# neonnnnn/nimfm

Measured on AMD Instinct MI355X. Metric: SGD training samples/sec/epoch, higher is better.
Workload: dtype f64

## Files before the change

nimfm_amd/csrc/mb.h:

```cpp
#pragma once
#include <functional>
#include <vector>

#include "opt_views.h"
#include "plan.h"

namespace nfm {

struct MbWork {
  DevBuf Abuf;
  DevBuf rec;
  DevBuf partsA;
  DevBuf partsB;
  DevBuf Dtab;
  DevBuf Stab;
  DevBuf Ftab;
  DevBuf out_acc;
  DevBuf contrib;
  DevBuf itbuf;
  DevBuf hpart;
  DevBuf prox;
  bool use_graph = true;
  void* graph_exec = nullptr;
  uint64_t graph_plan_serial = 0;
  uint64_t graph_data_serial = 0;
  int graph_opt = -1;
  int64_t batch_begin = 0, batch_end = -1;
  std::function<int(int64_t)> after_batch;
  std::function<bool(int64_t)> is_sync;
  std::vector<void*> seg_execs;
  std::vector<int64_t> seg_cut;
  uint64_t seg_plan_serial = 0, seg_data_serial = 0;
  int seg_opt = -1;
  int64_t seg_key = -1;
// ... 17 lines not shown
```

nimfm_amd/csrc/mb_fm.hip:

```cpp
#include "mb_fm_kernels.h"

namespace nfm {

#define NFM_DECL(LL) \
  int mb_fm_run_L##LL(nfm_ctx* ctx, int opt_kind, bool gen, const CsrView& X, const ModelView& M, const OptView& O, const Plan& P, MbWork& W, int TA);
NFM_DECL(1) NFM_DECL(2) NFM_DECL(4) NFM_DECL(8) NFM_DECL(16) NFM_DECL(32) NFM_DECL(64)
#undef NFM_DECL


__global__ void k_schedule(OptView O, int fit_linear, int fit_intercept, const int64_t* __restrict__ bat_pos,
                           const double* __restrict__ it0p, double* __restrict__ Dtab ,
                           double* __restrict__ Ftab ) {
  __shared__ double red[3][kBlock];
  const double it0 = *it0p;
  const int b = blockIdx.x;
  const int64_t p0 = bat_pos[b], p1 = bat_pos[b + 1];
  double dP = 1.0, dw = 1.0, d0 = 1.0;
  for (int64_t p = p0 + threadIdx.x; p < p1; p += kBlock) {
    const double it = it0 + (double)p;
    dP *= 1 - dev::get_eta(O.sched, O.eta0, O.power, O.beta, it) * O.beta;
    if (fit_linear) dw *= 1 - dev::get_eta(O.sched, O.eta0, O.power, O.alpha, it) * O.alpha;
    if (fit_intercept) d0 *= 1 - dev::get_eta(O.sched, O.eta0, O.power, O.alpha0, it) * O.alpha0;
  }
  red[0][threadIdx.x] = dP;
// ... 98 lines not shown
  const hipError_t e2 = hipGraphInstantiate(&exec, graph, nullptr, nullptr, 0);
  (void)hipGraphDestroy(graph);
  NFM_HIP_CHECK(e2);
  seg_execs.push_back(exec);
  seg_cut.push_back(b);
  NFM_HIP_CHECK(hipGraphLaunch(exec, ctx->stream));
  return NFM_OK;
}
int MbWork::seg_resume(nfm_ctx* ctx) {
  NFM_HIP_CHECK(hipStreamBeginCapture(ctx->stream, hipStreamCaptureModeThreadLocal));
  return NFM_OK;
}
MbWork::~MbWork() { drop_graph(); }

int mb_fm_epoch(nfm_ctx* ctx, int opt_kind, const CsrView& X, const ModelView& M, const OptView& O, const Plan& P, MbWork& W,
                int64_t it0, double* out2_host, uint64_t data_serial, bool defer_sync) {
  NFM_CHECK(M.kind == NFM_KIND_FM, NFM_ERR_UNSUPPORTED, "mb_fm_epoch: FM only");
  NFM_CHECK(M.degree <= dev::kMaxDeg, NFM_ERR_UNSUPPORTED, "mini-batch mode supports degree <= %d", dev::kMaxDeg);
  NFM_CHECK(M.Kp == 2 * M.L && M.Kp <= 128, NFM_ERR_UNSUPPORTED, "mini-batch mode: factor blocks of at most 128 (api.hip splits wider FMs)");
  hipStream_t st = ctx->stream;
  int TA = 0;
  for (int o = 0; o < M.nb; ++o) TA += M.deg_of(o) - 1;
  constexpr int kMinGroupsPerBlock = kWavesPerBlock;
  const void* before[] = {W.Abuf.p, W.rec.p, W.partsA.p, W.partsB.p, W.Dtab.p, W.Stab.p, W.Ftab.p, W.out_acc.p, W.itbuf.p, W.hpart.p, W.prox.p};
  NFM_TRY(W.Abuf.ensure(sizeof(double) * (size_t)std::max<int64_t>(P.max_batch, 1) * std::max(TA, 1) * M.Kp));
  NFM_TRY(W.rec.ensure(sizeof(SampleRec) * (size_t)std::max<int64_t>(P.max_batch, 1)));
  NFM_TRY(W.partsA.ensure(sizeof(PartA) * (size_t)(P.max_batch / 2 + 2)));
  NFM_TRY(W.partsB.ensure(sizeof(double) * 2 * (size_t)(P.max_unique / kMinGroupsPerBlock + P.max_batch / kWavesPerBlock + P.max_heavy / kWavesPerBlock + 6)));
  NFM_TRY(W.hpart.ensure(sizeof(double) * (size_t)std::max<int64_t>(P.max_segs, 1) * std::max(M.nb, 1) * (2 * M.Kp + 4)));
  NFM_TRY(W.Dtab.ensure(sizeof(double) * 4 * (size_t)(P.n_batches + 1)));
  NFM_TRY(W.Stab.ensure(sizeof(double) * 2 * (size_t)(P.n_batches + 1)));
  NFM_TRY(W.Ftab.ensure(sizeof(double) * 2 * kFtab * (size_t)(P.n_batches + 1)));
  NFM_TRY(W.out_acc.ensure(sizeof(double) * 2));
  NFM_TRY(W.itbuf.ensure(sizeof(double)));
  if (opt_kind == OPT_PSGD)
    NFM_TRY(W.prox.ensure(sizeof(double) * ((size_t)M.nb * M.da + (size_t)std::max(M.nb, 1) * M.Kp * (3 + 2 * 1024) + 8)));
  const void* after[] = {W.Abuf.p, W.rec.p, W.partsA.p, W.partsB.p, W.Dtab.p, W.Stab.p, W.Ftab.p, W.out_acc.p, W.itbuf.p, W.hpart.p, W.prox.p};
  for (size_t q = 0; q < sizeof(before) / sizeof(before[0]); ++q)
    if (before[q] != after[q]) W.drop_graph();
  hipLaunchKernelGGL(k_set_double, dim3(1), dim3(1), 0, st, W.itbuf.as<double>(), (double)it0);
  const bool want_graph = W.use_graph && !W.after_batch && !ctx->timing.enabled && !P.has_perm && P.n_batches >= 8;
  if (want_graph) {
    if (!W.graph_exec || W.graph_plan_serial != P.serial || W.graph_opt != opt_kind || W.graph_data_serial != data_serial) {
      W.drop_graph();
      hipGraph_t graph = nullptr;
      NFM_HIP_CHECK(hipStreamBeginCapture(st, hipStreamCaptureModeThreadLocal));
      const int rc = enqueue_epoch(ctx, opt_kind, X, M, O, P, W, TA);
      const hipError_t e = hipStreamEndCapture(st, &graph);
      if (rc != NFM_OK) {
        if (graph) (void)hipGraphDestroy(graph);
        return rc;
      }
      NFM_HIP_CHECK(e);
      hipGraphExec_t exec = nullptr;
      const hipError_t e2 = hipGraphInstantiate(&exec, graph, nullptr, nullptr, 0);
      (void)hipGraphDestroy(graph);
      NFM_HIP_CHECK(e2);
      W.graph_exec = exec;
      W.graph_plan_serial = P.serial;
      W.graph_data_serial = data_serial;
// ... 60 lines not shown
```

nimfm_amd/csrc/mb_fm_kernels.h:

```cpp
#pragma once
#include "fm_device.h"
#include "mb.h"

namespace nfm {

#ifndef NFM_WAVE_STAGE2
#define NFM_WAVE_STAGE2 1
#endif
#ifndef NFM_COL_MINW
#define NFM_COL_MINW 1
#endif
#ifndef NFM_COL_D3
#define NFM_COL_D3 1
#endif
#ifndef NFM_REG_NTSEL
#define NFM_REG_NTSEL 0
#endif
#ifndef NFM_ADA2_MINW
#define NFM_ADA2_MINW 2
#endif

struct SampleRec {
  double dL, etaP, etaw, yhat;
};
// ... 1 lines not shown
  double loss, viol, acc0, acc1;
};

static_assert(sizeof(SampleRec) == 32 && sizeof(PartA) == 32, "record layout");

constexpr int kFtab = 64;

struct RowArgs {
  CsrView X;
  ModelView M;
  OptView O;
  const int64_t* perm;
  int64_t begin, p0;
  int32_t len, use_stored, TA, nt;
  double it_b;
  const double* it0p;
  const double* scales;
  const double* scales_n;
  const int64_t* toff;
  const uint8_t* single;
  double* Abuf;
  SampleRec* rec;
  PartA* parts;
};

__device__ __forceinline__ void st_nt(double* p, double2 v) {
  dev::v2d_t w;
  w.x = v.x;
  w.y = v.y;
  __builtin_nontemporal_store(w, reinterpret_cast<dev::v2d_t*>(p));
}
__device__ __forceinline__ double2 ld_nt(const double* p) {
  const dev::v2d_t v = __builtin_nontemporal_load(reinterpret_cast<const dev::v2d_t*>(p));
  return double2{v.x, v.y};
}
template <bool NT>
__device__ __forceinline__ void st_row(double* p, double2 v) {
  if (NT) st_nt(p, v);
  else *reinterpret_cast<double2*>(p) = v;
}
template <bool NT>
__device__ __forceinline__ double2 ld_row(const double* p) {
  if (NT) return ld_nt(p);
  return *reinterpret_cast<const double2*>(p);
}
template <int L, int SPLIT, bool GEN, class PS>
// ... 423 lines not shown
    } else {
      const dev::AdaParams ps{O.G, O.N, O.eta0, O.eta0 * itp * O.beta};
      part += row_forward<L, SPLIT, GEN>(ps, X, M, q0, m, m_tot, slot, l, lane, valid, Arow, A1);
    }
  }
#pragma unroll
  for (int s = 1; s < LPS; s <<= 1) part += dev::shfl_xor_d(part, s);
  double dL, yh_w = 0.0;
  if (SPW == 1 && NFM_WAVE_STAGE2) {
    const double yh = wave_uniform(b0 + part);
    yh_w = yh;
    dL = wave_uniform(dev::loss_grad(O.loss, O.loss_param, y, yh));
    double r_acc0 = 0.0, r_acc1 = 0.0;
    if (OPT == OPT_SGD) {
      if (M.fit_intercept) {
        r_acc0 = eta_b * dL;
        r_acc1 = eta_b;
      }
    } else if (M.fit_intercept) {
      r_acc0 = dL;
      r_acc1 = dL * dL;
    }
    if (lane == 0) {
      if (valid) a.rec[pib] = SampleRec{dL, etaP, etaw, yh};
      s_dL[sib] = valid ? r_acc0 : 0.0;
      s_etaP[sib] = valid ? r_acc1 : 0.0;
    }
  } else {
  if (slot == 0 && l == 0) {
    s_y[sib] = y;
    s_yh[sib] = b0 + part;
  }
  __syncthreads();
  if (wv == 0) {
    double r_loss = 0.0, r_acc0 = 0.0, r_acc1 = 0.0;
    for (int t = lane; t < SPB; t += kWave) {
      const int pt = blockIdx.x * SPB + t;
      if (pt < a.len) {
        const double yt = s_y[t], yh = s_yh[t];
        const double dL = dev::loss_grad(O.loss, O.loss_param, yt, yh);
        r_loss += dev::loss_value(O.loss, O.loss_param, yt, yh);
        double etaP = 0.0, etaw = 0.0;
        if (OPT == OPT_SGD) {
          const double it = (a.it0p[0] + a.it_b) + (double)pt;
          etaP = dev::get_eta(O.sched, O.eta0, O.power, O.beta, it);
          etaw = dev::get_eta(O.sched, O.eta0, O.power, O.alpha, it);
          if (M.fit_intercept) {
            const double eta0 = dev::get_eta(O.sched, O.eta0, O.power, O.alpha0, it);
            r_acc0 += eta0 * dL;
            r_acc1 += eta0;
          }
        } else if (M.fit_intercept) {
          r_acc0 += dL;
          r_acc1 += dL * dL;
        }
        a.rec[pt] = SampleRec{dL, etaP, etaw, yh};
        s_dL[t] = dL;
        s_etaP[t] = etaP;
        s_etaw[t] = etaw;
      }
    }
    r_loss = dev::wave_sum(r_loss);
    r_acc0 = dev::wave_sum(r_acc0);
    r_acc1 = dev::wave_sum(r_acc1);
    if (lane == 0) {
      s_part[0] = r_loss;
      s_part[2] = r_acc0;
      s_part[3] = r_acc1;
    }
  }
  __syncthreads();
  dL = s_dL[sib];
  etaP = s_etaP[sib];
  etaw = s_etaw[sib];
  }
  double r_viol = 0.0;
  if (HELD && a.single != nullptr) {
    const double sP = OPT == OPT_SGD ? a.scales[0] : 1.0, sw = OPT == OPT_SGD ? a.scales[1] : 1.0;
    const double sPn = OPT == OPT_SGD ? a.scales_n[0] : 1.0, swn = OPT == OPT_SGD ? a.scales_n[1] : 1.0;
// ... 191 lines not shown
    a1.x += tx;
    a1.y += ty;
    a2.x += tx * tx;
    a2.y += ty * ty;
    __builtin_amdgcn_sched_barrier(0);
  }
#pragma unroll
  for (int s = 16; s < kWave; s <<= 1) {
    a1.x += dev::shfl_xor_d(a1.x, s);
    a1.y += dev::shfl_xor_d(a1.y, s);
    a2.x += dev::shfl_xor_d(a2.x, s);
    a2.y += dev::shfl_xor_d(a2.y, s);
  }
  if (valid && slot == 0) *reinterpret_cast<double2*>(a.Abuf + (size_t)pib * a.TA * M.Kp + eoff) = a1;
  if (slot == 0) part += (a1.x * a1.x - a2.x) / 2 + (a1.y * a1.y - a2.y) / 2;
  part = dev::wave_sum(part);
  if (lane == 0) s_part[sib][half] = part;
  __syncthreads();
  double b0 = M.sc[SC_INTERCEPT];
  if (M.fit_intercept) b0 = -O.eta0 * O.gsc[0] / (sqrt(O.gsc[1]) + O.eta0 * itp * O.alpha0);
  const double yh = wave_uniform(b0 + (s_part[sib][0] + s_part[sib][1]));
  const double dL = wave_uniform(dev::loss_grad(O.loss, O.loss_param, y, yh));
  if (half == 0 && lane == 0) {
    if (valid) a.rec[pib] = SampleRec{dL, 0.0, 0.0, yh};
    s_acc0[sib] = (valid && M.fit_intercept) ? dL : 0.0;
    s_acc1[sib] = (valid && M.fit_intercept) ? dL * dL : 0.0;
  }
  asm volatile("" : "+v"(jq), "+v"(fq), "+v"(xq));
  double r_viol = 0.0;
#ifndef NFM_ADA2_V
#define NFM_ADA2_V 8
#endif
  constexpr int V = NFM_ADA2_V;
#pragma unroll
  for (int u0 = 0; u0 < NU; u0 += V) {
    int f[V], j[V];
    double xv[V];
    double2 po[V];
#pragma unroll
    for (int u = 0; u < V; ++u) {
      f[u] = lane_bcast_i<SPLIT>(fq, u0 + u, slot);
      j[u] = lane_bcast_i<SPLIT>(jq, u0 + u, slot);
      xv[u] = lane_bcast_d<SPLIT>(xq, u0 + u, slot);
    }
    if (O.track_viol) {
#pragma unroll
      for (int u = 0; u < V; ++u) {
// ... 59 lines not shown
  int64_t begin, p0;
  int32_t len_i, nS;
  const int32_t* ucol;
  const int64_t* uptr;
  const int32_t* ucol_s;
  const int64_t* ubeg_s;
  const int32_t* ucnt_s;
  const int32_t* tpos;
  const double* tx;
  int64_t u0, u1;
  const double* scales_b;
  const double* scales_n;
  const double* Dtab_b;
  const double* Ftab_b;
  const double* Abuf;
  const SampleRec* rec;
  double* parts;
  const PartA* partsA;
  const double* parts_prev;
  double* out_acc;
  double it_b, len;
  const double* it0p;
  int32_t TA, use_stored, nA, n_prev;
};

struct WAcc {
  double a0 = 0.0, a1 = 0.0;
};

template <int OPT, bool GEN, int TU, int LG, int MODE>
__device__ __forceinline__ double col_block(const ColArgs& a, size_t e, int deg, int slot, int l, int64_t t0, int64_t t1,
                                            double sP, double sPn, double fP, bool do_w, WAcc& wacc, double c_total = 0.0,
                                            double* hp = nullptr, int64_t nseg = 0, int PW = 0, int seg_stride = 0) {
  const ModelView& M = a.M;
  const OptView& O = a.O;
  double viol = 0.0;
  double2 stored = {0.0, 0.0}, g2 = {0.0, 0.0}, n2 = {0.0, 0.0}, p;
  if (OPT == OPT_SGD) {
    stored = dev::ld_stream(M.P + e);
    p.x = sP * stored.x;
    p.y = sP * stored.y;
  } else if (OPT == OPT_PSGD) {
    stored = dev::ld_stream(M.P + e);
    p = stored;
  } else {
    g2 = dev::ld_stream(O.G + e);
// ... 965 lines not shown
      s1[f] = load_stage(h1[f]);
    }
#pragma unroll
    for (int f = 0; f < NF; ++f) finish(h0[f], s0[f], G[f]);
#pragma unroll
    for (int f = 0; f < NF; ++f) {
      h0[f] = h1[f];
      h1[f] = h2[f];
      s0[f] = s1[f];
    }
  }
  viol = dev::wave_sum(viol);
  if (lane == 0) red[0][wv] = viol;
  __syncthreads();
  if (threadIdx.x == 0) {
    double v = 0.0;
    for (int w_ = 0; w_ < kWavesPerBlock; ++w_) v += red[0][w_];
    a.parts[a.nS + blockIdx.x] = v;
  }
  if (!closer) return;
  col_closer<OPT>(a, red);
}

__global__ void k_epoch_close(const double* __restrict__ parts, int n, double* __restrict__ out_acc);

template <int L, int SPLIT, int OPT, bool GEN>
static void launch_row(hipStream_t st, const RowArgs& ra, int mode, int n_cu, int* n_blocks) {
  const bool sing = ra.single != nullptr;
  constexpr int SPW = kWave / (L * SPLIT);
  const int nA = (ra.len + kWavesPerBlock * SPW - 1) / (kWavesPerBlock * SPW);
  *n_blocks = nA;
  constexpr bool CAN_HOLD = held_entries<L, SPLIT>() > 0;
  constexpr bool CAN_REG = CAN_HOLD && !GEN && OPT == OPT_SGD && L * SPLIT == kWave;
  if (CAN_REG && mode == 2 && ra.nt)
    hipLaunchKernelGGL((k_row_phase<L, SPLIT, OPT, GEN, (CAN_REG ? 4 : 0), false>), dim3(nA), dim3(kBlock), 0, st, ra);
  else if (CAN_REG && mode == 2)
    hipLaunchKernelGGL((k_row_phase<L, SPLIT, OPT, GEN, (CAN_REG ? 2 : 0), false>), dim3(nA), dim3(kBlock), 0, st, ra);
  else if (CAN_HOLD && mode == 3)
    hipLaunchKernelGGL((k_row_phase<L, SPLIT, OPT, GEN, (CAN_HOLD ? 3 : 0), false>), dim3(nA), dim3(kBlock), 0, st, ra);
  else if (CAN_HOLD && mode >= 1)
    hipLaunchKernelGGL((k_row_phase<L, SPLIT, OPT, GEN, (CAN_HOLD ? 1 : 0), false>), dim3(nA), dim3(kBlock), 0, st, ra);
  else if (sing && !GEN)
    hipLaunchKernelGGL((k_row_phase<L, SPLIT, OPT, GEN, 0, !GEN>), dim3(nA), dim3(kBlock), 0, st, ra);
  else
    hipLaunchKernelGGL((k_row_phase<L, SPLIT, OPT, GEN, 0, false>), dim3(nA), dim3(kBlock), 0, st, ra);
}

static int held_capacity(int L, int s) {
  const int lps = L * s;
  const int e = lps >= kWave ? 1 : (lps >= 8 ? (kWave / lps > 4 ? 4 : kWave / lps) : 0);
  return e * lps;
}

template <int L, int OPT, bool GEN>
static int run_batches(nfm_ctx* ctx, const CsrView& X, const ModelView& M, const OptView& O, const Plan& P, MbWork& W,
                       int TA) {
  constexpr int R = kWave / L;
  hipStream_t st = ctx->stream;
  const double* Stab = W.Stab.as<double>();
  const double* Dtab = W.Dtab.as<double>();
  const double* it0p = W.itbuf.as<double>();
  const double avg_row = X.n > 0 ? (double)X.nnz / (double)X.n + M.n_aug : 0.0;
  const size_t partsB_half = W.partsB.bytes / sizeof(double) / 2;
  const char* tu_env = getenv("NFM_TU");
  const int tu = tu_env ? atoi(tu_env) : 2;
  const bool have_singles = !GEN && P.use_singles;
  static const int stream_env = getenv("NFM_STREAM") ? atoi(getenv("NFM_STREAM")) : -1;
  const size_t table_bytes = sizeof(double) * (size_t)M.nb * M.da * M.Kp * (OPT == OPT_ADAGRAD ? 3 : 1);
  const bool stream_rows = stream_env >= 0 ? stream_env != 0 : (have_singles && table_bytes > ((size_t)384 << 20));
  static const bool env_kernel = getenv("NFM_SINGLES_KERNEL") && atoi(getenv("NFM_SINGLES_KERNEL")) != 0;
  const bool singles_in_row = have_singles && !env_kernel;
  const bool singles_in_col = have_singles && !singles_in_row;
  int n_prev = 0;
  const int64_t b_first = std::min(W.batch_begin, P.n_batches), b_last = W.batch_end < 0 ? P.n_batches : std::min(W.batch_end, P.n_batches);
  for (int64_t b = b_first; b < b_last; ++b) {
    const int64_t p0 = P.bat_pos[b];
    const int len = (int)(P.bat_pos[b + 1] - p0);
    const int use_stored = (OPT == OPT_PSGD || (OPT == OPT_ADAGRAD && P.first_singleton && b == 0)) ? 1 : 0;
    const double it_b = OPT == OPT_PSGD ? (double)b : (double)p0;
    constexpr int ROPT = OPT == OPT_PSGD ? OPT_ADAGRAD : OPT;
    const int split = choose_split(L, len, avg_row, ctx->n_cu);
    auto mode_for = [&](int s_used) {
      static const bool held_on = !(getenv("NFM_HELD") && atoi(getenv("NFM_HELD")) == 0);
      static const bool reg_on = !(getenv("NFM_NQ") && atoi(getenv("NFM_NQ")) == 0);
      if (!held_on || held_capacity(L, s_used) == 0 || M.nb == 0) return 0;
      if (X.max_row + M.n_aug > held_capacity(L, s_used)) return 3;
      if (!GEN && reg_on && OPT == OPT_SGD && singles_in_row && L * s_used == kWave) return 2;
      return 1;
    };
    int nA;
    {
      RowArgs ra{X, M, O, P.has_perm ? P.perm.as<int64_t>() : nullptr, P.begin, p0, len, use_stored, TA, stream_rows ? 1 : 0, it_b, it0p,
                 OPT == OPT_SGD ? Stab + 2 * b : M.sc, OPT == OPT_SGD ? Stab + 2 * (b + 1) : M.sc,
                 singles_in_row ? P.toff.as<int64_t>() : nullptr,
                 singles_in_row ? P.single.as<uint8_t>() : nullptr, W.Abuf.as<double>(), W.rec.as<SampleRec>(),
                 W.partsA.as<PartA>()};
      TimedLaunch tl(ctx, "row_phase");
      int s_used;
      static const bool ada2_on = !(getenv("NFM_ADA2") && atoi(getenv("NFM_ADA2")) == 0);
      if (OPT == OPT_ADAGRAD && !GEN && L == 32 && ada2_on && singles_in_row && !use_stored && X.max_row + M.n_aug <= 64) {
        nA = (len + 1) / 2;
        if (stream_rows)
          hipLaunchKernelGGL((k_row_phase_ada2<OPT_ADAGRAD, true>), dim3(nA), dim3(kBlock), 0, st, ra);
        else
          hipLaunchKernelGGL((k_row_phase_ada2<OPT_ADAGRAD, false>), dim3(nA), dim3(kBlock), 0, st, ra);
        s_used = 2;
      } else
      if (R >= 16 && split >= 16) { launch_row<L, (R >= 16 ? 16 : R), ROPT, GEN>(st, ra, mode_for(R >= 16 ? 16 : R), ctx->n_cu, &nA); s_used = R >= 16 ? 16 : R; }
      else if (R >= 8 && split >= 8) { launch_row<L, (R >= 8 ? 8 : R), ROPT, GEN>(st, ra, mode_for(R >= 8 ? 8 : R), ctx->n_cu, &nA); s_used = R >= 8 ? 8 : R; }
      else if (R >= 4 && split >= 4) { launch_row<L, (R >= 4 ? 4 : R), ROPT, GEN>(st, ra, mode_for(R >= 4 ? 4 : R), ctx->n_cu, &nA); s_used = R >= 4 ? 4 : R; }
      else if (R >= 2 && split >= 2) { launch_row<L, (R >= 2 ? 2 : R), ROPT, GEN>(st, ra, mode_for(R >= 2 ? 2 : R), ctx->n_cu, &nA); s_used = R >= 2 ? 2 : R; }
      else { launch_row<L, 1, ROPT, GEN>(st, ra, mode_for(1), ctx->n_cu, &nA); s_used = 1; }
      (void)s_used;
    }
    const int64_t u0 = P.bat_uoff[b], u1 = P.bat_uoff[b + 1];
    const int per_block = kWavesPerBlock * R;
    int nB = (int)((u1 - u0 + per_block - 1) / per_block);
    static const bool col_pipe_env = !(getenv("NFM_COL_PIPE") && atoi(getenv("NFM_COL_PIPE")) == 0);
    const bool col_pipe = col_pipe_env && !GEN && M.nb == 1 && OPT != OPT_PSGD;
    static const int col_occ = [] {
      int nb_ = 0, np_ = 0;
      if (hipOccupancyMaxActiveBlocksPerMultiprocessor(&nb_, k_col_phase<L, OPT, GEN, 2, true>, kBlock, 0) != hipSuccess || nb_ < 1) nb_ = 8;
      if (!GEN && OPT != OPT_PSGD && col_pipe_env &&
          hipOccupancyMaxActiveBlocksPerMultiprocessor(&np_, k_col_sparse<L, (OPT == OPT_PSGD ? OPT_SGD : OPT)>, kBlock, 0) == hipSuccess && np_ >= 1)
        nb_ = np_;
      return nb_;
    }();
    static const int col_wg_per_cu = getenv("NFM_COL_WG") ? atoi(getenv("NFM_COL_WG")) : col_occ;
    static const int cap_sets = getenv("NFM_COL_CAP_SETS") ? atoi(getenv("NFM_COL_CAP_SETS")) : 4;
    const bool nB_capped = tu == 2 && col_wg_per_cu > 0 && nB > cap_sets * ctx->n_cu * col_wg_per_cu;
    if (nB_capped) nB = ctx->n_cu * col_wg_per_cu;
    nB += 1;
    const int nS = singles_in_col ? (len + kWavesPerBlock - 1) / kWavesPerBlock : 0;
    double* parts_cur = W.partsB.as<double>() + (b & 1) * partsB_half;
    const double* parts_prev = W.partsB.as<double>() + ((b + 1) & 1) * partsB_half;
    {
      ColArgs ca{X, M, O, P.has_perm ? P.perm.as<int64_t>() : nullptr, singles_in_col ? P.toff.as<int64_t>() : nullptr,
                 singles_in_col ? P.single.as<uint8_t>() : nullptr, P.begin, p0, len, nS,
                 P.ucol.as<int32_t>(), P.uptr.as<int64_t>(), P.ucol_s.as<int32_t>(), P.ubeg_s.as<int64_t>(), P.ucnt_s.as<int32_t>(),
                 P.tpos.as<int32_t>(), P.tx.as<double>(), u0, u1,
                 OPT == OPT_SGD ? Stab + 2 * b : M.sc, OPT == OPT_SGD ? Stab + 2 * (b + 1) : M.sc,
                 OPT == OPT_SGD ? Dtab + 4 * b : nullptr,
                 OPT == OPT_SGD ? W.Ftab.as<double>() + (size_t)b * 2 * kFtab : nullptr, W.Abuf.as<double>(),
                 W.rec.as<SampleRec>(), parts_cur, W.partsA.as<PartA>(), parts_prev, W.out_acc.as<double>(), it_b,
                 (double)len, it0p, TA, use_stored, nA, n_prev};
      if (nS > 0) {
        TimedLaunch tls(ctx, "singles");
        hipLaunchKernelGGL((k_singles<L, OPT>), dim3(nS), dim3(kBlock), 0, st, ca);
      }
      TimedLaunch tl(ctx, "col_phase");
      const bool strided = nB_capped;
      if (tu == 1 && OPT != OPT_PSGD)
        hipLaunchKernelGGL((k_col_phase<L, (OPT == OPT_PSGD ? OPT_SGD : OPT), GEN, 1, false>), dim3(nB), dim3(kBlock), 0, st, ca);
      else if (tu == 4 && OPT != OPT_PSGD)
        hipLaunchKernelGGL((k_col_phase<L, (OPT == OPT_PSGD ? OPT_SGD : OPT), GEN, 4, false>), dim3(nB), dim3(kBlock), 0, st, ca);
      else if (strided && col_pipe)
        hipLaunchKernelGGL((k_col_sparse<L, (OPT == OPT_PSGD ? OPT_SGD : OPT)>), dim3(nB), dim3(kBlock), 0, st, ca);
      else if (strided)
        hipLaunchKernelGGL((k_col_phase<L, OPT, GEN, 2, true>), dim3(nB), dim3(kBlock), 0, st, ca);
      else
        hipLaunchKernelGGL((k_col_phase<L, OPT, GEN, 2, false>), dim3(nB), dim3(kBlock), 0, st, ca);
    }
    int nH = 0;
    if (M.nb > 0 && P.bat_hoff[b + 1] > P.bat_hoff[b]) {
      const int PW = 2 * M.Kp + 4;
      HeavyArgs ha{P.hv_u.as<int64_t>(), P.hv_seg0.as<int64_t>(), P.bat_hoff[b], P.bat_hoff[b + 1], P.bat_soff[b],
                   P.bat_soff[b + 1], W.hpart.as<double>(), parts_cur + nS + nB, PW, 0};
      ColArgs ca{X, M, O, P.has_perm ? P.perm.as<int64_t>() : nullptr, nullptr, nullptr, P.begin, p0, len, nS,
                 P.ucol.as<int32_t>(), P.uptr.as<int64_t>(), P.ucol_s.as<int32_t>(), P.ubeg_s.as<int64_t>(), P.ucnt_s.as<int32_t>(),
                 P.tpos.as<int32_t>(), P.tx.as<double>(), u0, u1,
                 OPT == OPT_SGD ? Stab + 2 * b : M.sc, OPT == OPT_SGD ? Stab + 2 * (b + 1) : M.sc,
                 OPT == OPT_SGD ? Dtab + 4 * b : nullptr,
                 OPT == OPT_SGD ? W.Ftab.as<double>() + (size_t)b * 2 * kFtab : nullptr, W.Abuf.as<double>(),
                 W.rec.as<SampleRec>(), parts_cur, W.partsA.as<PartA>(), parts_prev, W.out_acc.as<double>(), it_b,
                 (double)len, it0p, TA, use_stored, nA, n_prev};
      const int nsb = (int)((ha.s1 - ha.s0 + per_block - 1) / per_block);
      nH = (int)((ha.h1 - ha.h0 + kWavesPerBlock - 1) / kWavesPerBlock);
      {
        TimedLaunch tl(ctx, "heavy_partial");
        hipLaunchKernelGGL((k_heavy_partial<L, OPT, GEN>), dim3(nsb), dim3(kBlock), 0, st, ca, ha);
      }
      TimedLaunch tl(ctx, "heavy_apply");
      hipLaunchKernelGGL((k_heavy_apply<L, OPT, GEN>), dim3(nH), dim3(kBlock), 0, st, ca, ha);
    }
    n_prev = nB + nS + nH;
    if (OPT == OPT_PSGD && O.gradP == nullptr) launch_psgd_step(ctx, M, O, W, it0p, it_b);
    if (W.after_batch) {
      const bool cut = W.seg_recording && W.is_sync && W.is_sync(b);
      if (cut) NFM_TRY(W.seg_cut_here(ctx, b));
      NFM_TRY(W.after_batch(b));
      if (cut) NFM_TRY(W.seg_resume(ctx));
    }
  }
  if (b_last > b_first) {
    const double* parts_last = W.partsB.as<double>() + ((b_last - 1) & 1) * partsB_half;
    hipLaunchKernelGGL(k_epoch_close, dim3(1), dim3(kBlock), 0, st, parts_last, n_prev, W.out_acc.as<double>());
  }
  NFM_HIP_CHECK(hipGetLastError());
// ... 5 lines not shown
```

nimfm_amd/csrc/plan.h:

```cpp
#pragma once
#include "common.h"

namespace nfm {

struct Plan {
  uint64_t serial = 0;
  uint64_t ds_uid = 0;
  int64_t ds_nnz = -1;
  int64_t begin = 0, end = 0, batch = 0;
  int n_aug = 0;
  bool first_singleton = false, has_perm = false, use_singles = false;
  int64_t n_batches = 0, U = 0, T = 0, TM = 0, max_batch = 0, max_unique = 0;
  std::vector<int64_t> bat_pos;
  std::vector<int64_t> bat_uoff;
  DevBuf perm;
  DevBuf bat_pos_dev;
  DevBuf ucol;
  DevBuf uptr;
  DevBuf ucol_s;
  DevBuf ubeg_s;
  DevBuf ucnt_s;
  DevBuf tpos;
  DevBuf tx;
  DevBuf tq;
  DevBuf toff;
  DevBuf single;
  int64_t H = 0, HS = 0;
  std::vector<int64_t> bat_hoff;
  std::vector<int64_t> bat_soff;
  int64_t max_heavy = 0, max_segs = 0;
  DevBuf hv_u;
  DevBuf hv_seg0;
  void release();
};

struct CscIndex {
  bool built = false, usable = false;
// ... 31 lines not shown
```

nimfm_amd/csrc/plan.hip:

```cpp
#include <hipcub/hipcub.hpp>
#include <type_traits>

#include <stdlib.h>

#include <atomic>

#include "plan.h"

namespace nfm {

void Plan::release() {
  perm.release();
  bat_pos_dev.release();
  ucol.release();
  uptr.release();
  ucol_s.release();
  ubeg_s.release();
  ucnt_s.release();
  tpos.release();
  tx.release();
  tq.release();
  toff.release();
  single.release();
  hv_u.release();
  hv_seg0.release();
  bat_hoff.clear();
  bat_soff.clear();
  H = HS = max_heavy = max_segs = 0;
  bat_pos.clear();
  bat_uoff.clear();
  n_batches = U = T = TM = 0;
}

__device__ __forceinline__ int64_t batch_of(int64_t rel, int64_t batch, int first_singleton) {
  if (first_singleton) return rel == 0 ? 0 : 1 + (rel - 1) / batch;
  return rel / batch;
}
__device__ __forceinline__ int64_t batch_start(int64_t b, int64_t batch, int first_singleton) {
  if (first_singleton) return b == 0 ? 0 : 1 + (b - 1) * batch;
  return b * batch;
}

__global__ void k_perm_range(int64_t ns, const int64_t* __restrict__ perm, int64_t n, unsigned long long* __restrict__ bad) {
  unsigned long long c = 0;
  for (int64_t r = (int64_t)blockIdx.x * blockDim.x + threadIdx.x; r < ns; r += (int64_t)gridDim.x * blockDim.x)
    c += (perm[r] < 0 || perm[r] >= n) ? 1 : 0;
  if (c) atomicAdd(bad, c);
}

__global__ void k_row_len(CsrView X, const int64_t* __restrict__ perm, int64_t begin, int64_t ns, int n_aug,
                          int64_t* __restrict__ len) {
  for (int64_t r = (int64_t)blockIdx.x * blockDim.x + threadIdx.x; r <= ns; r += (int64_t)gridDim.x * blockDim.x) {
    if (r == ns) {
// ... 881 lines not shown
template <class KeyT>
static int plan_build_t(nfm_ctx* ctx, hipStream_t st, const CsrView& X, int n_aug, const int64_t* perm_host, const int64_t* perm_given_dev,
                        int64_t begin, int64_t end, int64_t batch, bool first_singleton, bool want_tq, bool use_singles,
                        bool sort_by_count, Plan* out, CscIndex* csc, const FeistelKey* perm_key) {
  static std::atomic<uint64_t> g_serial{0};
  Plan& P = *out;
  P.release();
  P.serial = ++g_serial;
  const int64_t ns = end - begin;
  NFM_CHECK(ns >= 0 && begin >= 0 && (end <= X.n || perm_host || perm_given_dev), NFM_ERR_INVALID, "epoch range [%lld,%lld) outside [0,%lld)",
            (long long)begin, (long long)end, (long long)X.n);
  NFM_CHECK(batch >= 1, NFM_ERR_INVALID, "batch must be >= 1");
  P.begin = begin; P.end = end; P.batch = batch; P.n_aug = n_aug;
  P.first_singleton = first_singleton; P.has_perm = perm_host != nullptr || perm_given_dev != nullptr; P.use_singles = use_singles;
  P.bat_pos.clear();
  P.bat_pos.push_back(0);
  int64_t pos = 0;
  if (first_singleton && ns > 0) { pos = 1; P.bat_pos.push_back(1); }
  while (pos < ns) { pos = pos + batch < ns ? pos + batch : ns; P.bat_pos.push_back(pos); }
  P.n_batches = (int64_t)P.bat_pos.size() - 1;
  P.max_batch = 0;
  for (int64_t b = 0; b < P.n_batches; ++b) P.max_batch = std::max(P.max_batch, P.bat_pos[b + 1] - P.bat_pos[b]);
  P.bat_uoff.assign(P.n_batches + 1, 0);
  if (ns == 0) return NFM_OK;
  NFM_TRY(P.bat_pos_dev.alloc(sizeof(int64_t) * (P.n_batches + 1)));
  NFM_HIP_CHECK(hipMemcpyAsync(P.bat_pos_dev.p, P.bat_pos.data(), sizeof(int64_t) * (P.n_batches + 1), hipMemcpyHostToDevice, st));
  const int64_t* perm_dev = nullptr;
  if (perm_host || perm_given_dev) {
    NFM_TRY(P.perm.alloc(sizeof(int64_t) * ns));
    if (perm_given_dev)
      NFM_HIP_CHECK(hipMemcpyAsync(P.perm.p, perm_given_dev, sizeof(int64_t) * ns, hipMemcpyDeviceToDevice, st));
    else
      NFM_HIP_CHECK(hipMemcpyAsync(P.perm.p, perm_host + begin, sizeof(int64_t) * ns, hipMemcpyHostToDevice, st));
    perm_dev = P.perm.as<int64_t>();
  }
  DevBuf bad;
  if (perm_host) {
    NFM_TRY(bad.alloc(sizeof(unsigned long long)));
    NFM_HIP_CHECK(hipMemsetAsync(bad.p, 0, sizeof(unsigned long long), st));
    hipLaunchKernelGGL(k_perm_range, dim3(256 * 4), dim3(kBlock), 0, st, ns, perm_dev, X.n, bad.as<unsigned long long>());
    unsigned long long h_bad = 0;
    NFM_HIP_CHECK(hipMemcpyAsync(&h_bad, bad.p, sizeof(h_bad), hipMemcpyDeviceToHost, st));
    NFM_HIP_CHECK(hipStreamSynchronize(st));
    NFM_CHECK(h_bad == 0, NFM_ERR_INVALID, "%llu entries of the permutation are out of range [0,%lld)", h_bad, (long long)X.n);
  }
  DevBuf len, toff, tmp;
// ... 324 lines not shown
      hipcub::DoubleBuffer<uint32_t> udk(uk0.as<uint32_t>(), uk1.as<uint32_t>());
      hipcub::DoubleBuffer<uint32_t> udv(uv0.as<uint32_t>(), uv1.as<uint32_t>());
      hipLaunchKernelGGL(k_ukeys, dim3(grid1d(U)), dim3(kBlock), 0, st, U, ubatch.as<int64_t>(), P.uptr.as<int64_t>(), cbits,
                         uk0.as<uint32_t>(), uv0.as<uint32_t>());
      size_t ub = 0;
      NFM_HIP_CHECK(hipcub::DeviceRadixSort::SortPairs(nullptr, ub, udk, udv, (int)U, 0, cbits + bbits, st));
      NFM_TRY(utmp.alloc(ub));
      NFM_HIP_CHECK(hipcub::DeviceRadixSort::SortPairs(utmp.p, ub, udk, udv, (int)U, 0, cbits + bbits, st));
      order = udv.Current();
    }
    hipLaunchKernelGGL(k_usorted, dim3(grid1d(U)), dim3(kBlock), 0, st, U, order, P.ucol.as<int32_t>(),
                       P.uptr.as<int64_t>(), P.ucol_s.as<int32_t>(), P.ubeg_s.as<int64_t>(), P.ucnt_s.as<int32_t>(),
                       n_heavy.as<unsigned long long>());
  }
  std::vector<int64_t> first(P.n_batches);
  NFM_HIP_CHECK(hipMemcpyAsync(first.data(), bfu.p, sizeof(int64_t) * P.n_batches, hipMemcpyDeviceToHost, st));
  NFM_HIP_CHECK(hipMemcpyAsync(&h_heavy, n_heavy.p, sizeof(h_heavy), hipMemcpyDeviceToHost, st));
  NFM_HIP_CHECK(hipStreamSynchronize(st));
  P.bat_uoff[P.n_batches] = U;
  for (int64_t b = P.n_batches - 1; b >= 0; --b) P.bat_uoff[b] = first[b] != none ? first[b] : P.bat_uoff[b + 1];
  }
  P.max_unique = 0;
  for (int64_t b = 0; b < P.n_batches; ++b) P.max_unique = std::max(P.max_unique, P.bat_uoff[b + 1] - P.bat_uoff[b]);
  P.bat_hoff.assign(P.n_batches + 1, 0);
  P.bat_soff.assign(P.n_batches + 1, 0);
  if (U > 0 && h_heavy == 0) {
    NFM_TRY(P.hv_u.alloc(sizeof(int64_t)));
    NFM_TRY(P.hv_seg0.alloc(sizeof(int64_t)));
  } else if (U > 0) {
    DevBuf hflag, nseg, hidx, segoff, uoff_dev, hoff_dev, soff_dev;
    NFM_TRY(hflag.alloc(sizeof(int64_t) * (U + 1))); NFM_TRY(nseg.alloc(sizeof(int64_t) * (U + 1)));
    NFM_TRY(hidx.alloc(sizeof(int64_t) * (U + 1))); NFM_TRY(segoff.alloc(sizeof(int64_t) * (U + 1)));
    hipLaunchKernelGGL(k_heavy_flags, dim3(grid1d(U + 1)), dim3(kBlock), 0, st, U, P.uptr.as<int64_t>(), hflag.as<int64_t>(),
                       nseg.as<int64_t>());
    tmp_bytes = 0;
    NFM_HIP_CHECK(hipcub::DeviceScan::ExclusiveSum(nullptr, tmp_bytes, hflag.as<int64_t>(), hidx.as<int64_t>(), (int)(U + 1), st));
    NFM_TRY(tmp.alloc(tmp_bytes));
    NFM_HIP_CHECK(hipcub::DeviceScan::ExclusiveSum(tmp.p, tmp_bytes, hflag.as<int64_t>(), hidx.as<int64_t>(), (int)(U + 1), st));
    NFM_HIP_CHECK(hipcub::DeviceScan::ExclusiveSum(tmp.p, tmp_bytes, nseg.as<int64_t>(), segoff.as<int64_t>(), (int)(U + 1), st));
    NFM_TRY(uoff_dev.alloc(sizeof(int64_t) * (P.n_batches + 1)));
    NFM_TRY(hoff_dev.alloc(sizeof(int64_t) * (P.n_batches + 1)));
    NFM_TRY(soff_dev.alloc(sizeof(int64_t) * (P.n_batches + 1)));
    NFM_HIP_CHECK(hipMemcpyAsync(uoff_dev.p, P.bat_uoff.data(), sizeof(int64_t) * (P.n_batches + 1), hipMemcpyHostToDevice, st));
    hipLaunchKernelGGL(k_gather_i64, dim3(grid1d(P.n_batches + 1)), dim3(kBlock), 0, st, P.n_batches + 1, hidx.as<int64_t>(),
                       uoff_dev.as<int64_t>(), hoff_dev.as<int64_t>());
    hipLaunchKernelGGL(k_gather_i64, dim3(grid1d(P.n_batches + 1)), dim3(kBlock), 0, st, P.n_batches + 1, segoff.as<int64_t>(),
// ... 71 lines not shown
```

Measured before the change: 83.36 million.

## Add software-pipelined column kernel for long-touch columns with compact dL buffer

Adds k_col_long, a column-phase kernel that prefetches headers, metadata, records and factor rows several columns ahead and keeps a ring of Abuf rows, so latency is hidden when each column is touched many times. The row phase now also writes a compact per-sample dL buffer, and for schedules where eta can be recomputed on device the kernel reads only dL instead of the full SampleRec. The kernel is chosen by a heuristic (strided grid, L==32, mean touches per column at least 4) using per-batch touch offsets computed at plan time. The cost is an extra store per sample, an extra host sync during planning, and a larger register footprint.

```diff
diff --git a/nimfm_amd/csrc/mb.h b/nimfm_amd/csrc/mb.h
--- a/nimfm_amd/csrc/mb.h
+++ b/nimfm_amd/csrc/mb.h
@@ -10,6 +10,7 @@
 struct MbWork {
   DevBuf Abuf;
   DevBuf rec;
+  DevBuf dLbuf;
   DevBuf partsA;
   DevBuf partsB;
   DevBuf Dtab;
diff --git a/nimfm_amd/csrc/mb_fm.hip b/nimfm_amd/csrc/mb_fm.hip
--- a/nimfm_amd/csrc/mb_fm.hip
+++ b/nimfm_amd/csrc/mb_fm.hip
@@ -144,9 +144,10 @@
   int TA = 0;
   for (int o = 0; o < M.nb; ++o) TA += M.deg_of(o) - 1;
   constexpr int kMinGroupsPerBlock = kWavesPerBlock;
-  const void* before[] = {W.Abuf.p, W.rec.p, W.partsA.p, W.partsB.p, W.Dtab.p, W.Stab.p, W.Ftab.p, W.out_acc.p, W.itbuf.p, W.hpart.p, W.prox.p};
+  const void* before[] = {W.Abuf.p, W.rec.p, W.partsA.p, W.partsB.p, W.Dtab.p, W.Stab.p, W.Ftab.p, W.out_acc.p, W.itbuf.p, W.hpart.p, W.prox.p, W.dLbuf.p};
   NFM_TRY(W.Abuf.ensure(sizeof(double) * (size_t)std::max<int64_t>(P.max_batch, 1) * std::max(TA, 1) * M.Kp));
   NFM_TRY(W.rec.ensure(sizeof(SampleRec) * (size_t)std::max<int64_t>(P.max_batch, 1)));
+  NFM_TRY(W.dLbuf.ensure(sizeof(double) * (size_t)std::max<int64_t>(P.max_batch, 1)));
   NFM_TRY(W.partsA.ensure(sizeof(PartA) * (size_t)(P.max_batch / 2 + 2)));
   NFM_TRY(W.partsB.ensure(sizeof(double) * 2 * (size_t)(P.max_unique / kMinGroupsPerBlock + P.max_batch / kWavesPerBlock + P.max_heavy / kWavesPerBlock + 6)));
   NFM_TRY(W.hpart.ensure(sizeof(double) * (size_t)std::max<int64_t>(P.max_segs, 1) * std::max(M.nb, 1) * (2 * M.Kp + 4)));
@@ -157,7 +158,7 @@
   NFM_TRY(W.itbuf.ensure(sizeof(double)));
   if (opt_kind == OPT_PSGD)
     NFM_TRY(W.prox.ensure(sizeof(double) * ((size_t)M.nb * M.da + (size_t)std::max(M.nb, 1) * M.Kp * (3 + 2 * 1024) + 8)));
-  const void* after[] = {W.Abuf.p, W.rec.p, W.partsA.p, W.partsB.p, W.Dtab.p, W.Stab.p, W.Ftab.p, W.out_acc.p, W.itbuf.p, W.hpart.p, W.prox.p};
+  const void* after[] = {W.Abuf.p, W.rec.p, W.partsA.p, W.partsB.p, W.Dtab.p, W.Stab.p, W.Ftab.p, W.out_acc.p, W.itbuf.p, W.hpart.p, W.prox.p, W.dLbuf.p};
   for (size_t q = 0; q < sizeof(before) / sizeof(before[0]); ++q)
     if (before[q] != after[q]) W.drop_graph();
   hipLaunchKernelGGL(k_set_double, dim3(1), dim3(1), 0, st, W.itbuf.as<double>(), (double)it0);
diff --git a/nimfm_amd/csrc/mb_fm_kernels.h b/nimfm_amd/csrc/mb_fm_kernels.h
--- a/nimfm_amd/csrc/mb_fm_kernels.h
+++ b/nimfm_amd/csrc/mb_fm_kernels.h
@@ -47,6 +47,7 @@
   double* Abuf;
   SampleRec* rec;
   PartA* parts;
+  double* dLbuf;
 };
 
 __device__ __forceinline__ void st_nt(double* p, double2 v) {
@@ -516,7 +517,10 @@
       r_acc1 = dL * dL;
     }
     if (lane == 0) {
-      if (valid) a.rec[pib] = SampleRec{dL, etaP, etaw, yh};
+      if (valid) {
+        a.rec[pib] = SampleRec{dL, etaP, etaw, yh};
+        a.dLbuf[pib] = dL;
+      }
       s_dL[sib] = valid ? r_acc0 : 0.0;
       s_etaP[sib] = valid ? r_acc1 : 0.0;
     }
@@ -549,6 +553,7 @@
           r_acc1 += dL * dL;
         }
         a.rec[pt] = SampleRec{dL, etaP, etaw, yh};
+        a.dLbuf[pt] = dL;
         s_dL[t] = dL;
         s_etaP[t] = etaP;
         s_etaw[t] = etaw;
@@ -786,7 +791,10 @@
   const double yh = wave_uniform(b0 + (s_part[sib][0] + s_part[sib][1]));
   const double dL = wave_uniform(dev::loss_grad(O.loss, O.loss_param, y, yh));
   if (half == 0 && lane == 0) {
-    if (valid) a.rec[pib] = SampleRec{dL, 0.0, 0.0, yh};
+    if (valid) {
+      a.rec[pib] = SampleRec{dL, 0.0, 0.0, yh};
+      a.dLbuf[pib] = dL;
+    }
     s_acc0[sib] = (valid && M.fit_intercept) ? dL : 0.0;
     s_acc1[sib] = (valid && M.fit_intercept) ? dL * dL : 0.0;
   }
@@ -892,6 +900,7 @@
   double it_b, len;
   const double* it0p;
   int32_t TA, use_stored, nA, n_prev;
+  const double* dLbuf;
 };
 
 struct WAcc {
@@ -1903,6 +1912,271 @@
   col_closer<OPT>(a, red);
 }
 
+struct LongRow {
+  double2 st, g2, n2;
+};
+struct LongHdr {
+  int cnt, j, t0;
+};
+struct LongMeta {
+  int pib;
+  double x;
+};
+struct LongRec {
+  double dL, etaP, etaw;
+};
+
+#ifndef NFM_COL_LONG_D
+#define NFM_COL_LONG_D 4
+#endif
+#ifndef NFM_COL_LONG_MINW
+#define NFM_COL_LONG_MINW 4
+#endif
+constexpr double kColLongMean = 4.0;
+template <int L, int OPT, int D, bool COMPACT>
+__global__ __launch_bounds__(kBlock, NFM_COL_LONG_MINW) void k_col_long(ColArgs a) {
+  static_assert(OPT == OPT_SGD || OPT == OPT_ADAGRAD, "SGD / AdaGrad");
+  constexpr int R = kWave / L;
+  constexpr int DD = D < L ? D : L;
+  static_assert(L % DD == 0, "chunks tile a block");
+  __shared__ double red[5][kBlock];
+  const ModelView& M = a.M;
+  const OptView& O = a.O;
+  const int lane = threadIdx.x & (kWave - 1), wv = threadIdx.x >> 6;
+  const int g = lane / L, l = lane % L;
+  const int gbase = lane - l;
+  const bool closer = blockIdx.x == gridDim.x - 1;
+  const int64_t stride = (int64_t)(gridDim.x - 1) * kWavesPerBlock * R;
+  double viol = 0.0;
+  double sP = 1.0, sPn = 1.0, sw = 1.0, swn = 1.0;
+  if (OPT == OPT_SGD) {
+    sP = a.scales_b[0];
+    sw = a.scales_b[1];
+    sPn = a.scales_n[0];
+    swn = a.scales_n[1];
+  }
+  const double itp = (a.it0p[0] + a.it_b) - 1.0;
+  const double tmpP = O.eta0 * itp * O.beta;
+  const size_t a_stride = (size_t)a.TA * M.Kp;
+  auto load_hdr = [&](int64_t uu) {
+    LongHdr h{0, 0, 0};
+    if (uu < a.u1) {
+      h.cnt = a.ucnt_s[uu];
+      h.j = a.ucol_s[uu];
+      h.t0 = (int)a.ubeg_s[uu];
+      if (h.cnt > kHeavyTouches) h.cnt = 0;
+    }
+    return h;
+  };
+  auto load_row = [&](const LongHdr& h) {
+    LongRow s{};
+    if (h.cnt > 0) {
+      const size_t e = M.row(0, h.j) * M.Kp + 2 * l;
+      if (OPT == OPT_SGD) {
+        s.st = dev::ld_stream(M.P + e);
+      } else {
+        s.g2 = dev::ld_stream(O.G + e);
+        s.n2 = dev::ld_stream(O.N + e);
+        if (a.use_stored || O.track_viol) s.st = dev::ld_stream(M.P + e);
+      }
+    }
+    return s;
+  };
+  auto load_meta = [&](const LongHdr& h, int tb) {
+    LongMeta m{0, 0.0};
+    if (tb + l < h.cnt) {
+      m.pib = a.tpos[h.t0 + tb + l];
+      m.x = a.tx[h.t0 + tb + l];
+    }
+    return m;
+  };
+  auto eta_of = [&](double reg, double it) {
+    switch (O.sched) {
+      case NFM_SCHED_CONSTANT:
+        return O.eta0;
+      case NFM_SCHED_OPTIMAL:
+        return O.eta0 / (1.0 + O.eta0 * reg * it);
+      case NFM_SCHED_INVSCALING:
+        return O.eta0 / it;
+      default:
+        return 1.0 / (reg * it);
+    }
+  };
+  auto load_rec = [&](int pib) {
+    LongRec r{0.0, 0.0, 0.0};
+    if (COMPACT) {
+      r.dL = a.dLbuf[pib];
+      if (OPT == OPT_SGD) {
+        const double it = (a.it0p[0] + a.it_b) + (double)pib;
+        r.etaP = eta_of(O.beta, it);
+        r.etaw = eta_of(O.alpha, it);
+      }
+    } else {
+      const SampleRec* p = a.rec + pib;
+      r.dL = p->dL;
+      if (OPT == OPT_SGD) {
+        r.etaP = p->etaP;
+        r.etaw = p->etaw;
+      }
+    }
+    return r;
+  };
+  auto load_A = [&](int pib) { return *reinterpret_cast<const double2*>(a.Abuf + (size_t)pib * a_stride + 2 * l); };
+  auto add_touch = [&](const SampleRec& r, double2 A1, double x, double2 p, bool do_w, double2& acc, double2& accn, double& seta,
+                       WAcc& wacc) {
+    const double dAx = x * (A1.x - p.x * x);
+    const double dAy = x * (A1.y - p.y * x);
+    if (OPT == OPT_SGD) {
+      acc.x += r.etaP * (r.dL * dAx);
+      acc.y += r.etaP * (r.dL * dAy);
+      seta += r.etaP;
+      if (do_w) {
+        wacc.a0 += r.etaw * (r.dL * x);
+        wacc.a1 += r.etaw;
+      }
+    } else {
+      const double gx = r.dL * dAx, gy = r.dL * dAy;
+      acc.x += gx;
+      acc.y += gy;
+      accn.x += gx * gx;
+      accn.y += gy * gy;
+      if (do_w) {
+        const double gw = r.dL * x;
+        wacc.a0 += gw;
+        wacc.a1 += gw * gw;
+      }
+    }
+  };
+  int64_t u = closer ? a.u1 : a.u0 + ((int64_t)blockIdx.x * kWavesPerBlock + wv) * R + g;
+  LongHdr h0 = load_hdr(u), h1 = load_hdr(u + stride), h2 = load_hdr(u + 2 * stride);
+  LongMeta m0 = load_meta(h0, 0), m1 = load_meta(h1, 0);
+  LongRec r0 = load_rec(m0.pib);
+  LongRow s0 = load_row(h0);
+  double2 ring[DD];
+#pragma unroll
+  for (int q = 0; q < DD; ++q) ring[q] = load_A(__shfl(m0.pib, gbase + q, kWave));
+  for (; u < a.u1; u += stride) {
+    const LongHdr h3 = load_hdr(u + 3 * stride);
+    const LongMeta m2 = load_meta(h2, 0);
+    const LongRow s1 = load_row(h1);
+    const int cnt = h0.cnt;
+    const int64_t j = h0.j;
+    const size_t e = M.row(0, j) * M.Kp + 2 * l;
+    const bool do_w = M.fit_linear && j < M.d;
+    double fP = 1.0, fw = 1.0, wt = 0.0, gw = 0.0, nw = 0.0;
+    if (cnt > 0) {
+      if (OPT == OPT_SGD) touch_factors(a, cnt, fP, fw);
+      if (do_w) {
+        wt = M.w[j];
+        if (OPT == OPT_ADAGRAD) {
+          gw = O.Gw[j];
+          nw = O.Nw[j];
+        }
+      }
+    }
+    double2 stored = s0.st, g2 = s0.g2, n2 = s0.n2, p = {0.0, 0.0};
+    if (cnt > 0) {
+      if (OPT == OPT_SGD) {
+        p.x = sP * stored.x;
+        p.y = sP * stored.y;
+      } else if (a.use_stored) {
+        p = stored;
+      } else {
+        p.x = dev::adagrad_param(g2.x, n2.x, O.eta0, tmpP);
+        p.y = dev::adagrad_param(g2.y, n2.y, O.eta0, tmpP);
+        if (O.track_viol) {
+          viol += fabs(stored.x - p.x) + fabs(stored.y - p.y);
+          dev::st_stream(M.P + e, p);
+        }
+      }
+    }
+    double2 acc = {0.0, 0.0}, accn = {0.0, 0.0};
+    double seta = 0.0;
+    WAcc wacc;
+    auto walk = [&](const LongMeta& mc, const LongRec& rc, int bcnt, int npib) {
+      int cb = 0;
+      do {
+        const bool last = cb + DD >= bcnt;
+#pragma unroll
+        for (int q = 0; q < DD; ++q) {
+          const int tl = cb + q;
+          SampleRec r;
+          const double x = dev::shfl_d(mc.x, gbase + tl);
+          r.dL = dev::shfl_d(rc.dL, gbase + tl);
+          r.etaP = OPT == OPT_SGD ? dev::shfl_d(rc.etaP, gbase + tl) : 0.0;
+          r.etaw = OPT == OPT_SGD ? dev::shfl_d(rc.etaw, gbase + tl) : 0.0;
+          r.yhat = 0.0;
+          if (tl < bcnt) add_touch(r, ring[q], x, p, do_w, acc, accn, seta, wacc);
+          ring[q] = load_A(__shfl(last ? npib : mc.pib, gbase + (last ? q : tl + DD), kWave));
+        }
+        cb += DD;
+      } while (cb < bcnt);
+    };
+    if (cnt <= L) {
+      walk(m0, r0, cnt, m1.pib);
+    } else {
+      LongMeta mc = m0;
+      LongRec rc = r0;
+      for (int tb = 0; tb < cnt; tb += L) {
+        const bool more = tb + L < cnt;
+        const LongMeta mn = more ? load_meta(h0, tb + L) : m1;
+        walk(mc, rc, cnt - tb < L ? cnt - tb : L, mn.pib);
+        mc = mn;
+        if (more) rc = load_rec(mc.pib);
+      }
+    }
+    r0 = load_rec(m1.pib);
+    if (cnt > 0) {
+      const double c = OPT == OPT_SGD ? dev::touch_div((double)cnt, O.touch_cap) : (double)cnt;
+      if (OPT == OPT_SGD) {
+        viol += fabs((acc.x + seta * O.beta * p.x) / c) + fabs((acc.y + seta * O.beta * p.y) / c);
+        stored.x = stored.x * fP - (acc.x / c) / sPn;
+        stored.y = stored.y * fP - (acc.y / c) / sPn;
+        dev::st_stream(M.P + e, stored);
+        if (do_w) {
+          const double wj = sw * wt;
+          if (l == 0) {
+            viol += fabs((wacc.a0 + wacc.a1 * O.alpha * wj) / c);
+            M.w[j] = wt * fw - (wacc.a0 / c) / swn;
+          }
+        }
+      } else {
+        g2.x += acc.x;
+        g2.y += acc.y;
+        n2.x += dev::ada_norm_inc(acc.x, accn.x, O.ada_cross);
+        n2.y += dev::ada_norm_inc(acc.y, accn.y, O.ada_cross);
+        dev::st_stream(O.G + e, g2);
+        dev::st_stream(O.N + e, n2);
+        if (do_w && l == 0) {
+          if (!a.use_stored) {
+            const double wj = -O.eta0 * gw / (itp * O.eta0 * O.alpha + sqrt(nw));
+            viol += fabs(wt - wj);
+            M.w[j] = wj;
+          }
+          O.Gw[j] = gw + wacc.a0;
+          O.Nw[j] = nw + dev::ada_norm_inc(wacc.a0, wacc.a1, O.ada_cross);
+        }
+      }
+    }
+    h0 = h1;
+    h1 = h2;
+    h2 = h3;
+    m0 = m1;
+    m1 = m2;
+    s0 = s1;
+  }
+  viol = dev::wave_sum(viol);
+  if (lane == 0) red[0][wv] = viol;
+  __syncthreads();
+  if (threadIdx.x == 0) {
+    double v = 0.0;
+    for (int w_ = 0; w_ < kWavesPerBlock; ++w_) v += red[0][w_];
+    a.parts[a.nS + blockIdx.x] = v;
+  }
+  if (!closer) return;
+  col_closer<OPT>(a, red);
+}
+
 __global__ void k_epoch_close(const double* __restrict__ parts, int n, double* __restrict__ out_acc);
 
 template <int L, int SPLIT, int OPT, bool GEN>
@@ -1946,6 +2220,13 @@
   const char* tu_env = getenv("NFM_TU");
   const int tu = tu_env ? atoi(tu_env) : 2;
   const bool have_singles = !GEN && P.use_singles;
+  const char* long_env = getenv("NFM_COL_LONG");
+  const int col_long_knob = long_env ? (atoi(long_env) != 0 ? 1 : 0) : -1;
+  const char* compact_env = getenv("NFM_COL_LONG_COMPACT");
+  const bool col_long_compact = !(compact_env && atoi(compact_env) == 0) &&
+                                (OPT != OPT_SGD || O.power == 1.0 || (O.sched != NFM_SCHED_OPTIMAL && O.sched != NFM_SCHED_INVSCALING));
+  const char* grid_env = getenv("NFM_COL_GRID");
+  const int col_grid = grid_env ? atoi(grid_env) : 0;
   static const int stream_env = getenv("NFM_STREAM") ? atoi(getenv("NFM_STREAM")) : -1;
   const size_t table_bytes = sizeof(double) * (size_t)M.nb * M.da * M.Kp * (OPT == OPT_ADAGRAD ? 3 : 1);
   const bool stream_rows = stream_env >= 0 ? stream_env != 0 : (have_singles && table_bytes > ((size_t)384 << 20));
@@ -1975,7 +2256,7 @@
                  OPT == OPT_SGD ? Stab + 2 * b : M.sc, OPT == OPT_SGD ? Stab + 2 * (b + 1) : M.sc,
                  singles_in_row ? P.toff.as<int64_t>() : nullptr,
                  singles_in_row ? P.single.as<uint8_t>() : nullptr, W.Abuf.as<double>(), W.rec.as<SampleRec>(),
-                 W.partsA.as<PartA>()};
+                 W.partsA.as<PartA>(), W.dLbuf.as<double>()};
       TimedLaunch tl(ctx, "row_phase");
       int s_used;
       static const bool ada2_on = !(getenv("NFM_ADA2") && atoi(getenv("NFM_ADA2")) == 0);
@@ -2009,8 +2290,8 @@
     }();
     static const int col_wg_per_cu = getenv("NFM_COL_WG") ? atoi(getenv("NFM_COL_WG")) : col_occ;
     static const int cap_sets = getenv("NFM_COL_CAP_SETS") ? atoi(getenv("NFM_COL_CAP_SETS")) : 4;
-    const bool nB_capped = tu == 2 && col_wg_per_cu > 0 && nB > cap_sets * ctx->n_cu * col_wg_per_cu;
-    if (nB_capped) nB = ctx->n_cu * col_wg_per_cu;
+    const bool nB_capped = tu == 2 && ((col_wg_per_cu > 0 && nB > cap_sets * ctx->n_cu * col_wg_per_cu) || (col_grid > 0 && nB > col_grid));
+    if (nB_capped) nB = col_grid > 0 ? std::min(nB, col_grid) : ctx->n_cu * col_wg_per_cu;
     nB += 1;
     const int nS = singles_in_col ? (len + kWavesPerBlock - 1) / kWavesPerBlock : 0;
     double* parts_cur = W.partsB.as<double>() + (b & 1) * partsB_half;
@@ -2024,17 +2305,24 @@
                  OPT == OPT_SGD ? Dtab + 4 * b : nullptr,
                  OPT == OPT_SGD ? W.Ftab.as<double>() + (size_t)b * 2 * kFtab : nullptr, W.Abuf.as<double>(),
                  W.rec.as<SampleRec>(), parts_cur, W.partsA.as<PartA>(), parts_prev, W.out_acc.as<double>(), it_b,
-                 (double)len, it0p, TA, use_stored, nA, n_prev};
+                 (double)len, it0p, TA, use_stored, nA, n_prev, W.dLbuf.as<double>()};
       if (nS > 0) {
         TimedLaunch tls(ctx, "singles");
         hipLaunchKernelGGL((k_singles<L, OPT>), dim3(nS), dim3(kBlock), 0, st, ca);
       }
       TimedLaunch tl(ctx, "col_phase");
       const bool strided = nB_capped;
+      const int64_t nt_b = (int64_t)P.bat_toff.size() > b + 1 ? P.bat_toff[b + 1] - P.bat_toff[b] : 0;
+      const bool col_long = col_pipe && tu == 2 && col_long_knob != 0 &&
+                            (col_long_knob == 1 || (strided && L == 32 && (double)nt_b >= kColLongMean * (double)(u1 - u0)));
       if (tu == 1 && OPT != OPT_PSGD)
         hipLaunchKernelGGL((k_col_phase<L, (OPT == OPT_PSGD ? OPT_SGD : OPT), GEN, 1, false>), dim3(nB), dim3(kBlock), 0, st, ca);
       else if (tu == 4 && OPT != OPT_PSGD)
         hipLaunchKernelGGL((k_col_phase<L, (OPT == OPT_PSGD ? OPT_SGD : OPT), GEN, 4, false>), dim3(nB), dim3(kBlock), 0, st, ca);
+      else if (col_long && col_long_compact)
+        hipLaunchKernelGGL((k_col_long<L, (OPT == OPT_PSGD ? OPT_SGD : OPT), NFM_COL_LONG_D, true>), dim3(nB), dim3(kBlock), 0, st, ca);
+      else if (col_long)
+        hipLaunchKernelGGL((k_col_long<L, (OPT == OPT_PSGD ? OPT_SGD : OPT), NFM_COL_LONG_D, false>), dim3(nB), dim3(kBlock), 0, st, ca);
       else if (strided && col_pipe)
         hipLaunchKernelGGL((k_col_sparse<L, (OPT == OPT_PSGD ? OPT_SGD : OPT)>), dim3(nB), dim3(kBlock), 0, st, ca);
       else if (strided)
@@ -2054,7 +2342,7 @@
                  OPT == OPT_SGD ? Dtab + 4 * b : nullptr,
                  OPT == OPT_SGD ? W.Ftab.as<double>() + (size_t)b * 2 * kFtab : nullptr, W.Abuf.as<double>(),
                  W.rec.as<SampleRec>(), parts_cur, W.partsA.as<PartA>(), parts_prev, W.out_acc.as<double>(), it_b,
-                 (double)len, it0p, TA, use_stored, nA, n_prev};
+                 (double)len, it0p, TA, use_stored, nA, n_prev, W.dLbuf.as<double>()};
       const int nsb = (int)((ha.s1 - ha.s0 + per_block - 1) / per_block);
       nH = (int)((ha.h1 - ha.h0 + kWavesPerBlock - 1) / kWavesPerBlock);
       {
diff --git a/nimfm_amd/csrc/plan.h b/nimfm_amd/csrc/plan.h
--- a/nimfm_amd/csrc/plan.h
+++ b/nimfm_amd/csrc/plan.h
@@ -13,6 +13,7 @@
   int64_t n_batches = 0, U = 0, T = 0, TM = 0, max_batch = 0, max_unique = 0;
   std::vector<int64_t> bat_pos;
   std::vector<int64_t> bat_uoff;
+  std::vector<int64_t> bat_toff;
   DevBuf perm;
   DevBuf bat_pos_dev;
   DevBuf ucol;
diff --git a/nimfm_amd/csrc/plan.hip b/nimfm_amd/csrc/plan.hip
--- a/nimfm_amd/csrc/plan.hip
+++ b/nimfm_amd/csrc/plan.hip
@@ -29,6 +29,7 @@
   H = HS = max_heavy = max_segs = 0;
   bat_pos.clear();
   bat_uoff.clear();
+  bat_toff.clear();
   n_batches = U = T = TM = 0;
 }
 
@@ -956,6 +957,7 @@
   P.max_batch = 0;
   for (int64_t b = 0; b < P.n_batches; ++b) P.max_batch = std::max(P.max_batch, P.bat_pos[b + 1] - P.bat_pos[b]);
   P.bat_uoff.assign(P.n_batches + 1, 0);
+  P.bat_toff.assign(P.n_batches + 1, 0);
   if (ns == 0) return NFM_OK;
   NFM_TRY(P.bat_pos_dev.alloc(sizeof(int64_t) * (P.n_batches + 1)));
   NFM_HIP_CHECK(hipMemcpyAsync(P.bat_pos_dev.p, P.bat_pos.data(), sizeof(int64_t) * (P.n_batches + 1), hipMemcpyHostToDevice, st));
@@ -1326,6 +1328,16 @@
   }
   P.max_unique = 0;
   for (int64_t b = 0; b < P.n_batches; ++b) P.max_unique = std::max(P.max_unique, P.bat_uoff[b + 1] - P.bat_uoff[b]);
+  {
+    DevBuf uoff_dev, toff_dev;
+    NFM_TRY(uoff_dev.alloc(sizeof(int64_t) * (P.n_batches + 1)));
+    NFM_TRY(toff_dev.alloc(sizeof(int64_t) * (P.n_batches + 1)));
+    NFM_HIP_CHECK(hipMemcpyAsync(uoff_dev.p, P.bat_uoff.data(), sizeof(int64_t) * (P.n_batches + 1), hipMemcpyHostToDevice, st));
+    hipLaunchKernelGGL(k_gather_i64, dim3(grid1d(P.n_batches + 1)), dim3(kBlock), 0, st, P.n_batches + 1, P.uptr.as<int64_t>(),
+                       uoff_dev.as<int64_t>(), toff_dev.as<int64_t>());
+    NFM_HIP_CHECK(hipMemcpyAsync(P.bat_toff.data(), toff_dev.p, sizeof(int64_t) * (P.n_batches + 1), hipMemcpyDeviceToHost, st));
+    NFM_HIP_CHECK(hipStreamSynchronize(st));
+  }
   P.bat_hoff.assign(P.n_batches + 1, 0);
   P.bat_soff.assign(P.n_batches + 1, 0);
   if (U > 0 && h_heavy == 0) {
```

Result: faster. 85.29 million, median of 6 (+2.3%).
